# rclarey/torrent

Measured on AMD Instinct MI355X. Metric: verified GB/s (SHA-1 pieces, HBM-resident), higher is better.
Workload: dtype u32

## Files before the change

torrent_amd/csrc/tv_sha256.h:

```cpp
#pragma once
#include <stdint.h>

#if defined(__HIP_DEVICE_COMPILE__)
#define TV_SHA256_FN __device__ __forceinline__
#define TV_XOR3(a, b, c) __builtin_amdgcn_bitop3_b32((a), (b), (c), 0x96)
#define TV_CH(e, f, g) __builtin_amdgcn_bitop3_b32((e), (f), (g), 0xCA)
#define TV_MAJ(a, b, c) __builtin_amdgcn_bitop3_b32((a), (b), (c), 0xE8)
#define TV_ROR(x, n) __builtin_rotateright32((x), (n))
#else
#if defined(__HIPCC__)
#define TV_SHA256_FN __host__ __device__ inline
#else
#define TV_SHA256_FN inline
#endif
#define TV_XOR3(a, b, c) ((a) ^ (b) ^ (c))
#define TV_CH(e, f, g) (((e) & (f)) | (~(e) & (g)))
#define TV_MAJ(a, b, c) (((a) & (b)) | ((a) & (c)) | ((b) & (c)))
#define TV_ROR(x, n) (((x) >> (n)) | ((x) << (32 - (n))))
#endif

namespace tv256 {

constexpr uint32_t kK[64] = {
    0x428a2f98u, 0x71374491u, 0xb5c0fbcfu, 0xe9b5dba5u, 0x3956c25bu, 0x59f111f1u, 0x923f82a4u, 0xab1c5ed5u,
    0xd807aa98u, 0x12835b01u, 0x243185beu, 0x550c7dc3u, 0x72be5d74u, 0x80deb1feu, 0x9bdc06a7u, 0xc19bf174u,
    0xe49b69c1u, 0xefbe4786u, 0x0fc19dc6u, 0x240ca1ccu, 0x2de92c6fu, 0x4a7484aau, 0x5cb0a9dcu, 0x76f988dau,
    0x983e5152u, 0xa831c66du, 0xb00327c8u, 0xbf597fc7u, 0xc6e00bf3u, 0xd5a79147u, 0x06ca6351u, 0x14292967u,
    0x27b70a85u, 0x2e1b2138u, 0x4d2c6dfcu, 0x53380d13u, 0x650a7354u, 0x766a0abbu, 0x81c2c92eu, 0x92722c85u,
    0xa2bfe8a1u, 0xa81a664bu, 0xc24b8b70u, 0xc76c51a3u, 0xd192e819u, 0xd6990624u, 0xf40e3585u, 0x106aa070u,
    0x19a4c116u, 0x1e376c08u, 0x2748774cu, 0x34b0bcb5u, 0x391c0cb3u, 0x4ed8aa4au, 0x5b9cca4fu, 0x682e6ff3u,
    0x748f82eeu, 0x78a5636fu, 0x84c87814u, 0x8cc70208u, 0x90befffau, 0xa4506cebu, 0xbef9a3f7u, 0xc67178f2u};

TV_SHA256_FN void iv(uint32_t h[8]) {
    h[0] = 0x6a09e667u; h[1] = 0xbb67ae85u; h[2] = 0x3c6ef372u; h[3] = 0xa54ff53au;
    h[4] = 0x510e527fu; h[5] = 0x9b05688cu; h[6] = 0x1f83d9abu; h[7] = 0x5be0cd19u;
}

TV_SHA256_FN void compress(const uint32_t h[8], uint32_t w[16], uint32_t out[8]) {
    uint32_t a = h[0], b = h[1], c = h[2], d = h[3], e = h[4], f = h[5], g = h[6], hh = h[7];
#pragma unroll
    for (int t = 0; t < 64; t++) {
        if (t >= 16) {
            const uint32_t x = w[(t + 1) & 15], y = w[(t + 14) & 15];
            const uint32_t s0 = TV_XOR3(TV_ROR(x, 7), TV_ROR(x, 18), x >> 3);
            const uint32_t s1 = TV_XOR3(TV_ROR(y, 17), TV_ROR(y, 19), y >> 10);
            w[t & 15] = w[t & 15] + s0 + w[(t + 9) & 15] + s1;
        }
        const uint32_t S1 = TV_XOR3(TV_ROR(e, 6), TV_ROR(e, 11), TV_ROR(e, 25));
        const uint32_t S0 = TV_XOR3(TV_ROR(a, 2), TV_ROR(a, 13), TV_ROR(a, 22));
        const uint32_t t1 = hh + S1 + TV_CH(e, f, g) + kK[t] + w[t & 15];
        const uint32_t t2 = S0 + TV_MAJ(a, b, c);
        hh = g; g = f; f = e; e = d + t1; d = c; c = b; b = a; a = t1 + t2;
    }
    const uint32_t r[8] = {a, b, c, d, e, f, g, hh};
#pragma unroll
    for (int i = 0; i < 8; i++) out[i] = h[i] + r[i];
}

}
```

torrent_amd/csrc/tv_v2_kernels.hip:

```cpp
#include <hip/hip_runtime.h>
#include <stdint.h>

#include "tv_block.h"
#include "tv_internal.h"
#include "tv_sha256.h"

namespace {

constexpr uint32_t kLeaf = 16384;
constexpr int kDepth = 3;

__device__ __forceinline__ uint32_t wave_min(uint32_t v) {
#pragma unroll
    for (int m = 32; m >= 1; m >>= 1) {
        const uint32_t o = (uint32_t)__shfl_xor((int)v, m, 64);
        v = o < v ? o : v;
    }
    return (uint32_t)__builtin_amdgcn_readfirstlane((int)v);
}

__device__ __forceinline__ uint32_t wave_max(uint32_t v) {
#pragma unroll
    for (int m = 32; m >= 1; m >>= 1) {
        const uint32_t o = (uint32_t)__shfl_xor((int)v, m, 64);
        v = o > v ? o : v;
    }
    return (uint32_t)__builtin_amdgcn_readfirstlane((int)v);
}

__device__ __forceinline__ void bswap_block(const uint4 (&r)[4], uint32_t w[16]) {
#pragma unroll
    for (int i = 0; i < 4; i++) {
        w[4 * i + 0] = bswap32(r[i].x);
        w[4 * i + 1] = bswap32(r[i].y);
        w[4 * i + 2] = bswap32(r[i].z);
        w[4 * i + 3] = bswap32(r[i].w);
    }
}

__device__ __forceinline__ void hash_leaf(const uint8_t* leaf, uint32_t len, bool active, uint32_t h[8]) {
    const uint32_t nb = active ? (uint32_t)nblocks(len) : 0;
    const uint32_t fast_end = wave_min(active ? len >> 6 : 0xFFFFFFFFu);
    const uint32_t end = wave_max(nb);
    if (active) {
        uint32_t w[16];
        tv256::iv(h);
        uint32_t b = 0;
        if (b < fast_end) {
            const uint32_t last = fast_end - 1;
            uint4 R[kDepth][4];
#pragma unroll
            for (int d = 0; d < kDepth; d++) load_block(leaf, b + d < last ? b + d : last, R[d]);
            for (;;) {
#pragma unroll
                for (int d = 0; d < kDepth; d++) {
                    bswap_block(R[d], w);
                    load_block(leaf, b + kDepth < last ? b + kDepth : last, R[d]);
                    tv256::compress(h, w, h);
                    if (++b >= fast_end) goto raw_done;
                }
            }
        }
    raw_done:
        for (; b < end; b++) {
            build_tail_block(leaf, len, b, w);
            uint32_t r[8];
            tv256::compress(h, w, r);
            if (b < nb) {
#pragma unroll
                for (int i = 0; i < 8; i++) h[i] = r[i];
            }
        }
    }
}

__device__ __forceinline__ void hash_pair(uint32_t w[16], uint32_t h[8]) {
    tv256::iv(h);
    tv256::compress(h, w, h);
    uint32_t pad[16] = {0x80000000u, 0, 0, 0, 0, 0, 0, 0, 0, 0, 0, 0, 0, 0, 0, 512u};
    tv256::compress(h, pad, h);
}

}

template <int MAP>
__global__ __launch_bounds__(256) void tv_v2_leaf_kernel(TvV2 p) {
    uint64_t t0 = 0, r0 = 0;
    if (p.clock && blockIdx.x == 0) {
        t0 = __builtin_amdgcn_s_memtime();
        r0 = __builtin_amdgcn_s_memrealtime();
    }
    const uint32_t logW = p.logW, W = 1u << logW;
    const uint64_t t = (uint64_t)blockIdx.x * 256u + threadIdx.x;
    uint64_t j;
    uint32_t k;
    if (MAP == TV_V2_MAP_LEAF) {
        j = t >> logW;
        k = (uint32_t)t & (W - 1u);
    } else {
        const uint32_t r = (uint32_t)t & ((64u << logW) - 1u);
        j = (t >> (6u + logW)) * 64u + (r & 63u);
        k = r >> 6;
    }
    const bool valid = j < p.n;
    const uint64_t bytes = valid ? p.piece_bytes[j] : 0;
    const uint32_t wj = valid ? p.tree_leaves[j] : 0;
    const bool in_tree = k < wj;
    const uint64_t lo = (uint64_t)k * kLeaf;
    const bool active = in_tree && lo < bytes;
    const uint32_t len = active ? (uint32_t)(bytes - lo < kLeaf ? bytes - lo : kLeaf) : 0;
    const uint64_t np = (uint64_t)p.n << logW;
    const uint64_t slot = (j << logW) + k;
    if (in_tree && !active) {
#pragma unroll
        for (int q = 0; q < 8; q++) p.nodes_a[q * np + slot] = 0;
    }
    uint32_t h[8];
    hash_leaf(p.data + j * p.stride + lo, len, active, h);
    if (active) {
#pragma unroll
        for (int q = 0; q < 8; q++) p.nodes_a[q * np + slot] = h[q];
    }
    if (p.clock && blockIdx.x == 0 && threadIdx.x == 0) {
        const uint64_t t1 = __builtin_amdgcn_s_memtime(), r1 = __builtin_amdgcn_s_memrealtime();
        reinterpret_cast<ulonglong2*>(p.clock)[0] = make_ulonglong2(t0, r0);
        reinterpret_cast<ulonglong2*>(p.clock)[1] = make_ulonglong2(t1, r1);
    }
}

__global__ __launch_bounds__(256) void tv_v2_level_kernel(TvV2 p, uint32_t level, uint32_t log_half) {
    const uint64_t t = (uint64_t)blockIdx.x * 256u + threadIdx.x;
    const uint64_t j = t >> log_half;
    const uint32_t i = (uint32_t)t & ((1u << log_half) - 1u);
    if (j >= p.n) return;
    if (i >= (p.tree_leaves[j] >> (level + 1u))) return;
    const uint64_t W = 1ull << p.logW, WB = W > 1 ? W / 2 : 1;
    const bool from_a = (level & 1u) == 0;
    const uint32_t* in = from_a ? p.nodes_a : p.nodes_b;
    uint32_t* out = from_a ? p.nodes_b : p.nodes_a;
    const uint64_t in_row = from_a ? W : WB, out_row = from_a ? WB : W;
    const uint64_t in_np = p.n * in_row, out_np = p.n * out_row;
    const uint64_t src = j * in_row + 2ull * i, dst = j * out_row + i;
    uint32_t w[16], h[8];
#pragma unroll
    for (int q = 0; q < 8; q++) {
        const uint2 v = *reinterpret_cast<const uint2*>(in + q * in_np + src);
        w[q] = v.x;
        w[8 + q] = v.y;
    }
    tv256::iv(h);
    tv256::compress(h, w, h);
    uint32_t pad[16] = {0x80000000u, 0, 0, 0, 0, 0, 0, 0, 0, 0, 0, 0, 0, 0, 0, 512u};
    tv256::compress(h, pad, h);
#pragma unroll
    for (int q = 0; q < 8; q++) out[q * out_np + dst] = h[q];
}

template <bool HASH>
__global__ __launch_bounds__(256) void tv_v2_finish_kernel(TvV2 p) {
    const uint32_t j = blockIdx.x * 256u + threadIdx.x;
    bool ok = j < p.n;
    if (ok) {
        const uint64_t W = 1ull << p.logW, WB = W > 1 ? W / 2 : 1;
        const uint32_t lw = 31u - (uint32_t)__builtin_clz(p.tree_leaves[j]);
        const bool in_a = (lw & 1u) == 0;
        const uint32_t* src = in_a ? p.nodes_a : p.nodes_b;
        const uint64_t row = in_a ? W : WB, np = p.n * row;
#pragma unroll
        for (int q = 0; q < 8; q++) {
            const uint32_t v = src[q * np + j * row];
            if (HASH) p.roots[(uint64_t)q * p.n + j] = v;
            else ok &= v == p.expect[(uint64_t)q * p.n + j];
        }
    }
    if (HASH) return;
    const uint64_t mask = __ballot(ok);
    if ((threadIdx.x & 63u) == 0 && (p.out_words == 0 || (j >> 6) < p.out_words)) {
        uint64_t bits = __builtin_bswap64(__builtin_bitreverse64(mask));
        if (p.avail64) bits &= p.avail64[j >> 6];
        p.out64[j >> 6] = bits;
    }
}

namespace {

__device__ __forceinline__ void list_emit(const TvV2List& p, uint32_t e, const uint32_t h[8]) {
    bool ok = true;
#pragma unroll
    for (int q = 0; q < 8; q++) ok &= h[q] == p.expect[(uint64_t)q * p.m + e];
    p.out_bytes[e] = ok ? 1 : 0;
}

__device__ __forceinline__ bool list_level(uint32_t (&s)[8][256], uint32_t t, uint32_t parents, uint32_t h[8]) {
    const bool par = t < parents;
    uint32_t w[16];
    if (par) {
#pragma unroll
        for (int q = 0; q < 8; q++) {
            const uint2 v = *reinterpret_cast<const uint2*>(&s[q][2 * t]);
            w[q] = v.x;
            w[8 + q] = v.y;
        }
    }
    __syncthreads();
    if (par) {
        hash_pair(w, h);
#pragma unroll
        for (int q = 0; q < 8; q++) s[q][t] = h[q];
    }
    __syncthreads();
    return par;
}

}

template <bool TILED>
__global__ __launch_bounds__(256) void tv_v2_list_kernel(TvV2List p) {
    __shared__ __attribute__((aligned(16))) uint32_t s_node[8][256];
    __shared__ __attribute__((aligned(16))) uint32_t s_root[8][256];
    __shared__ uint32_t s_lw[256];
    const uint32_t t = threadIdx.x;
    const uint32_t logW = p.logW, logT = logW < 8u ? logW : 8u;
    const uint32_t tiles = 1u << (logW - logT);
    const uint32_t e0 = blockIdx.x << (8u - logT);
    const uint32_t e = e0 + (t >> logT), kt = t & ((1u << logT) - 1u);
    const bool valid = e < p.m;
    const uint32_t bytes = valid ? p.bytes[e] : 0;
    const uint32_t we = valid ? p.widths[e] : 0;
    const uint8_t* row = p.data + (valid ? (uint64_t)p.rows[e] * p.stride : 0);
    if (kt == 0) s_lw[t >> logT] = valid ? 31u - (uint32_t)__builtin_clz(we) : 0xFFu;
    uint32_t h[8];
    for (uint32_t T = 0; T < (TILED ? tiles : 1u); T++) {
        const uint32_t k = (T << logT) + kt;
        const uint32_t lo = k * kLeaf;
        const bool active = k < we && lo < bytes;
        const uint32_t len = active ? (bytes - lo < kLeaf ? bytes - lo : kLeaf) : 0;
        hash_leaf(row + lo, len, active, h);
        if (!active) {
#pragma unroll
            for (int q = 0; q < 8; q++) h[q] = 0;
        }
        if (T == 0 && kt == 0 && we == 1) list_emit(p, e, h);
#pragma unroll
        for (int q = 0; q < 8; q++) s_node[q][t] = h[q];
        __syncthreads();
        for (uint32_t l = 0; l < logT; l++) {
            if (!list_level(s_node, t, 256u >> (l + 1u), h)) continue;
            const uint32_t sh = logT - l - 1u, g = t >> sh;
            if ((t & ((1u << sh) - 1u)) != 0) continue;
            if (T == 0 && s_lw[g] == l + 1u) list_emit(p, e0 + g, h);
            if (tiles > 1 && sh == 0) {
#pragma unroll
                for (int q = 0; q < 8; q++) s_root[q][T] = h[q];
            }
        }
    }
    if (TILED) __syncthreads();
    for (uint32_t l = 8; l < logW; l++)
        if (list_level(s_root, t, tiles >> (l - 7u), h) && t == 0 && s_lw[0] == l + 1u) list_emit(p, e0, h);
}

namespace {

__device__ __forceinline__ void column_store(const TvV2Col& p, uint32_t j, const uint32_t h[8]) {
    const uint64_t np = (uint64_t)p.n << p.logn, slot = ((uint64_t)j << p.logn) + p.col;
#pragma unroll
    for (int q = 0; q < 8; q++) p.nodes[q * np + slot] = h[q];
}

}

template <bool TILED>
__global__ __launch_bounds__(256) void tv_v2_column_kernel(TvV2Col p) {
    __shared__ __attribute__((aligned(16))) uint32_t s_node[8][256];
    __shared__ __attribute__((aligned(16))) uint32_t s_root[8][256];
    __shared__ uint32_t s_tg[256];
    uint64_t t0 = 0, r0 = 0;
    if (p.clock && blockIdx.x == 0) {
        t0 = __builtin_amdgcn_s_memtime();
        r0 = __builtin_amdgcn_s_memrealtime();
    }
    const uint32_t t = threadIdx.x;
    const uint32_t logc = p.logc, logT = logc < 8u ? logc : 8u;
    const uint32_t tiles = 1u << (logc - logT);
    const uint32_t j0 = blockIdx.x << (8u - logT);
    const uint32_t j = j0 + (t >> logT), kt = t & ((1u << logT) - 1u);
    const bool valid = j < p.n;
    const uint32_t bytes = valid ? p.piece_bytes[j] : 0;
    const uint32_t wj = valid ? p.tree_leaves[j] : 0;
    const uint64_t k0 = (uint64_t)p.col << logc;
    const bool reach = k0 < wj;
    const uint32_t lw = wj ? 31u - (uint32_t)__builtin_clz(wj) : 0u;
    const uint32_t target = lw < logc ? lw : logc;
    const uint8_t* row = p.data + (valid ? (uint64_t)j * p.stride : 0);
    if (kt == 0) s_tg[t >> logT] = reach ? target : 0xFFu;
    uint32_t h[8];
    for (uint32_t T = 0; T < (TILED ? tiles : 1u); T++) {
        const uint32_t kr = (T << logT) + kt;
        const uint64_t lo = (k0 + kr) * kLeaf;
        const bool active = k0 + kr < wj && lo < bytes;
        const uint32_t len = active ? (uint32_t)(bytes - lo < kLeaf ? bytes - lo : kLeaf) : 0;
        hash_leaf(row + (uint64_t)kr * kLeaf, len, active, h);
        if (!active) {
#pragma unroll
            for (int q = 0; q < 8; q++) h[q] = 0;
        }
        if (T == 0 && kt == 0 && reach && target == 0) column_store(p, j, h);
#pragma unroll
        for (int q = 0; q < 8; q++) s_node[q][t] = h[q];
        __syncthreads();
        for (uint32_t l = 0; l < logT; l++) {
            if (!list_level(s_node, t, 256u >> (l + 1u), h)) continue;
            const uint32_t sh = logT - l - 1u, g = t >> sh;
            if ((t & ((1u << sh) - 1u)) != 0) continue;
            if (T == 0 && s_tg[g] == l + 1u) column_store(p, j0 + g, h);
            if (tiles > 1 && sh == 0) {
#pragma unroll
                for (int q = 0; q < 8; q++) s_root[q][T] = h[q];
            }
        }
    }
    if (TILED) __syncthreads();
    for (uint32_t l = 8; l < logc; l++)
        if (list_level(s_root, t, tiles >> (l - 7u), h) && t == 0 && s_tg[0] == l + 1u) column_store(p, j0, h);
    if (p.clock && blockIdx.x == 0 && threadIdx.x == 0) {
        const uint64_t t1 = __builtin_amdgcn_s_memtime(), r1 = __builtin_amdgcn_s_memrealtime();
        reinterpret_cast<ulonglong2*>(p.clock)[0] = make_ulonglong2(t0, r0);
        reinterpret_cast<ulonglong2*>(p.clock)[1] = make_ulonglong2(t1, r1);
    }
}

template <bool CHECK>
__global__ __launch_bounds__(256) void tv_v2_block_kernel(TvV2Blocks p) {
    const uint32_t t = blockIdx.x * 256u + threadIdx.x;
    const bool active = t < p.m;
    const uint32_t row = active ? p.rows[t] : 0;
    const uint32_t leaf = active ? p.leaves[t] : 0;
    const uint32_t len = active ? p.lens[t] : 0;
    uint32_t h[8];
    hash_leaf(p.data + (uint64_t)row * p.stride + (uint64_t)leaf * kLeaf, len, active, h);
    if (CHECK) {
        bool ok = active;
        if (active) {
#pragma unroll
            for (int q = 0; q < 8; q++) ok &= h[q] == p.expect[(uint64_t)q * p.m + t];
        }
        const uint64_t mask = __ballot(ok);
        if ((threadIdx.x & 63u) == 0 && active) p.out64[t >> 6] = mask;
    } else if (active) {
#pragma unroll
        for (int q = 0; q < 8; q++) p.hashes[(uint64_t)q * p.m + t] = h[q];
    }
}

hipError_t tv_v2_launch_blocks(const TvV2Blocks& p, bool check, hipStream_t s, uint32_t* workgroups) {
    if (workgroups) *workgroups = 0;
    if (p.m == 0) return hipSuccess;
    if (p.m > TV_V2_BLOCKS_MAX_ITEMS) return hipErrorInvalidValue;
    const uint32_t grid = (p.m + 255u) / 256u;
    if (workgroups) *workgroups = grid;
    if (check) hipLaunchKernelGGL(tv_v2_block_kernel<true>, dim3(grid), dim3(256), 0, s, p);
    else hipLaunchKernelGGL(tv_v2_block_kernel<false>, dim3(grid), dim3(256), 0, s, p);
    return hipGetLastError();
}

hipError_t tv_v2_launch_column(const TvV2Col& p, hipStream_t s, uint32_t* workgroups) {
    if (workgroups) *workgroups = 0;
    if (p.n == 0) return hipSuccess;
    if (p.logc > TV_V2_COL_MAX_LOGC || (p.col >> p.logn) != 0) return hipErrorInvalidValue;
    const uint32_t logG = p.logc < 8u ? 8u - p.logc : 0u;
    const uint64_t grid = (((uint64_t)p.n - 1) >> logG) + 1;
    if (grid > 0x7FFFFFFFull) return hipErrorInvalidConfiguration;
    if (workgroups) *workgroups = (uint32_t)grid;
    if (p.logc > 8u) hipLaunchKernelGGL(tv_v2_column_kernel<true>, dim3((unsigned)grid), dim3(256), 0, s, p);
    else hipLaunchKernelGGL(tv_v2_column_kernel<false>, dim3((unsigned)grid), dim3(256), 0, s, p);
    return hipGetLastError();
}

hipError_t tv_v2_launch_leaves(const TvV2& p, hipStream_t s, uint32_t* workgroups) {
    if (workgroups) *workgroups = 0;
    if (p.n == 0) return hipSuccess;
    const uint64_t pieces = p.map == TV_V2_MAP_PIECE ? ((uint64_t)p.n + 63) / 64 * 64 : p.n;
    const uint64_t grid = ((pieces << p.logW) + 255) / 256;
    if (grid > 0x7FFFFFFFull) return hipErrorInvalidConfiguration;
    if (workgroups) *workgroups = (uint32_t)grid;
    if (p.map == TV_V2_MAP_PIECE)
        hipLaunchKernelGGL((tv_v2_leaf_kernel<TV_V2_MAP_PIECE>), dim3((unsigned)grid), dim3(256), 0, s, p);
    else
        hipLaunchKernelGGL((tv_v2_leaf_kernel<TV_V2_MAP_LEAF>), dim3((unsigned)grid), dim3(256), 0, s, p);
    return hipGetLastError();
}

hipError_t tv_v2_launch_level(const TvV2& p, uint32_t level, uint32_t maxlog, hipStream_t s) {
    if (p.n == 0 || level >= maxlog) return hipSuccess;
    const uint32_t log_half = maxlog - level - 1;
    const uint64_t grid = (((uint64_t)p.n << log_half) + 255) / 256;
    if (grid > 0x7FFFFFFFull) return hipErrorInvalidConfiguration;
    hipLaunchKernelGGL(tv_v2_level_kernel, dim3((unsigned)grid), dim3(256), 0, s, p, level, log_half);
    return hipGetLastError();
}

hipError_t tv_v2_launch_list(const TvV2List& p, hipStream_t s, uint32_t* workgroups) {
    if (workgroups) *workgroups = 0;
    if (p.m == 0) return hipSuccess;
    if (p.logW > TV_V2_LIST_MAX_LOGW) return hipErrorInvalidValue;
    const uint32_t logG = p.logW < 8u ? 8u - p.logW : 0u;
    const uint64_t grid = (((uint64_t)p.m - 1) >> logG) + 1;
    if (grid > 0x7FFFFFFFull) return hipErrorInvalidConfiguration;
    if (workgroups) *workgroups = (uint32_t)grid;
    if (p.logW > 8u) hipLaunchKernelGGL(tv_v2_list_kernel<true>, dim3((unsigned)grid), dim3(256), 0, s, p);
    else hipLaunchKernelGGL(tv_v2_list_kernel<false>, dim3((unsigned)grid), dim3(256), 0, s, p);
    return hipGetLastError();
}

hipError_t tv_v2_launch_finish(const TvV2& p, bool hash, hipStream_t s) {
    if (p.n == 0) return hipSuccess;
    const dim3 grid((p.n + 255) / 256);
    if (hash) hipLaunchKernelGGL((tv_v2_finish_kernel<true>), grid, dim3(256), 0, s, p);
    else hipLaunchKernelGGL((tv_v2_finish_kernel<false>), grid, dim3(256), 0, s, p);
    return hipGetLastError();
}
```

Before: 1442.

## Add lean single-buffer SHA-256 leaf path with in-round prefetch and occupancy hint

Adds a compress_lean variant that byte-swaps message words inside the first 16 rounds and issues the next block's load after round 15, once the raw registers are free. This lets the leaf kernel hold one block of prefetch instead of three. The leaf kernel defaults to depth 1 with a waves-per-EU attribute of 7, trading prefetch depth for more resident waves to hide HBM latency. Per-round asm fences and sched_barriers pin the instruction schedule, which may stop the compiler from interleaving work across rounds. The leaf-map slot index is also simplified to the thread id.

```diff
diff --git a/torrent_amd/csrc/tv_sha256.h b/torrent_amd/csrc/tv_sha256.h
--- a/torrent_amd/csrc/tv_sha256.h
+++ b/torrent_amd/csrc/tv_sha256.h
@@ -7,6 +7,11 @@
 #define TV_CH(e, f, g) __builtin_amdgcn_bitop3_b32((e), (f), (g), 0xCA)
 #define TV_MAJ(a, b, c) __builtin_amdgcn_bitop3_b32((a), (b), (c), 0xE8)
 #define TV_ROR(x, n) __builtin_rotateright32((x), (n))
+#define TV_ROUND_FENCE(a, e, w)                        \
+    do {                                               \
+        asm volatile("" : "+v"(a), "+v"(e), "+v"(w));  \
+        __builtin_amdgcn_sched_barrier(0);             \
+    } while (0)
 #else
 #if defined(__HIPCC__)
 #define TV_SHA256_FN __host__ __device__ inline
@@ -17,7 +22,9 @@
 #define TV_CH(e, f, g) (((e) & (f)) | (~(e) & (g)))
 #define TV_MAJ(a, b, c) (((a) & (b)) | ((a) & (c)) | ((b) & (c)))
 #define TV_ROR(x, n) (((x) >> (n)) | ((x) << (32 - (n))))
+#define TV_ROUND_FENCE(a, e, w) ((void)0)
 #endif
+#define TV_BSWAP(x) __builtin_bswap32(x)
 
 namespace tv256 {
 
@@ -57,4 +64,28 @@
     for (int i = 0; i < 8; i++) out[i] = h[i] + r[i];
 }
 
+template <bool SWAP, class After16>
+TV_SHA256_FN void compress_lean(uint32_t h[8], const uint32_t raw[16], uint32_t w[16], After16 after16) {
+    uint32_t a = h[0], b = h[1], c = h[2], d = h[3], e = h[4], f = h[5], g = h[6], hh = h[7];
+#pragma unroll
+    for (int t = 0; t < 64; t++) {
+        if (t < 16) {
+            w[t] = SWAP ? TV_BSWAP(raw[t]) : raw[t];
+        } else {
+            const uint32_t x = w[(t + 1) & 15], y = w[(t + 14) & 15];
+            const uint32_t s0 = TV_XOR3(TV_ROR(x, 7), TV_ROR(x, 18), x >> 3);
+            const uint32_t s1 = TV_XOR3(TV_ROR(y, 17), TV_ROR(y, 19), y >> 10);
+            w[t & 15] = w[t & 15] + s0 + w[(t + 9) & 15] + s1;
+        }
+        const uint32_t S1 = TV_XOR3(TV_ROR(e, 6), TV_ROR(e, 11), TV_ROR(e, 25));
+        const uint32_t S0 = TV_XOR3(TV_ROR(a, 2), TV_ROR(a, 13), TV_ROR(a, 22));
+        const uint32_t t1 = hh + S1 + TV_CH(e, f, g) + kK[t] + w[t & 15];
+        const uint32_t t2 = S0 + TV_MAJ(a, b, c);
+        hh = g; g = f; f = e; e = d + t1; d = c; c = b; b = a; a = t1 + t2;
+        if (t == 15) after16();
+        TV_ROUND_FENCE(a, e, w[t < 15 ? t : (t + 1) & 15]);
+    }
+    h[0] += a; h[1] += b; h[2] += c; h[3] += d; h[4] += e; h[5] += f; h[6] += g; h[7] += hh;
 }
+
+}
diff --git a/torrent_amd/csrc/tv_v2_kernels.hip b/torrent_amd/csrc/tv_v2_kernels.hip
--- a/torrent_amd/csrc/tv_v2_kernels.hip
+++ b/torrent_amd/csrc/tv_v2_kernels.hip
@@ -8,7 +8,17 @@
 namespace {
 
 constexpr uint32_t kLeaf = 16384;
-constexpr int kDepth = 3;
+#ifndef TV_V2_LEAF_DEPTH
+#define TV_V2_LEAF_DEPTH 1
+#endif
+#ifndef TV_V2_LEAF_WAVES
+#define TV_V2_LEAF_WAVES 7
+#endif
+#define TV_V2_WAVES __attribute__((amdgpu_waves_per_eu(TV_V2_LEAF_WAVES, TV_V2_LEAF_WAVES)))
+constexpr int kDepth = TV_V2_LEAF_DEPTH;
+constexpr int kWaves = TV_V2_LEAF_WAVES;
+constexpr int kListDepth = 3;
+static_assert(kDepth >= 1 && kDepth <= 3 && kWaves >= 1 && kWaves <= 8, "TV_V2_LEAF_DEPTH 1..3, TV_V2_LEAF_WAVES 1..8");
 
 __device__ __forceinline__ uint32_t wave_min(uint32_t v) {
 #pragma unroll
@@ -38,6 +48,7 @@
     }
 }
 
+template <int DEPTH>
 __device__ __forceinline__ void hash_leaf(const uint8_t* leaf, uint32_t len, bool active, uint32_t h[8]) {
     const uint32_t nb = active ? (uint32_t)nblocks(len) : 0;
     const uint32_t fast_end = wave_min(active ? len >> 6 : 0xFFFFFFFFu);
@@ -48,24 +59,43 @@
         uint32_t b = 0;
         if (b < fast_end) {
             const uint32_t last = fast_end - 1;
-            uint4 R[kDepth][4];
-#pragma unroll
-            for (int d = 0; d < kDepth; d++) load_block(leaf, b + d < last ? b + d : last, R[d]);
-            for (;;) {
-#pragma unroll
-                for (int d = 0; d < kDepth; d++) {
-                    bswap_block(R[d], w);
-                    load_block(leaf, b + kDepth < last ? b + kDepth : last, R[d]);
-                    tv256::compress(h, w, h);
-                    if (++b >= fast_end) goto raw_done;
+            if constexpr (DEPTH == 1) {
+                uint4 R[4];
+                load_block(leaf, 0, R);
+                const uint8_t* next = leaf;
+                do {
+                    next += b < last ? 64 : 0;
+                    tv256::compress_lean<true>(h, reinterpret_cast<const uint32_t*>(R), w,
+                                               [&] { load_block(next, 0, R); });
+                } while (++b < fast_end);
+            } else {
+                uint4 R[DEPTH][4];
+#pragma unroll
+                for (int d = 0; d < DEPTH; d++) load_block(leaf, b + d < last ? b + d : last, R[d]);
+                for (;;) {
+#pragma unroll
+                    for (int d = 0; d < DEPTH; d++) {
+                        bswap_block(R[d], w);
+                        load_block(leaf, b + DEPTH < last ? b + DEPTH : last, R[d]);
+                        tv256::compress(h, w, h);
+                        if (++b >= fast_end) goto raw_done;
+                    }
                 }
             }
         }
     raw_done:
         for (; b < end; b++) {
-            build_tail_block(leaf, len, b, w);
             uint32_t r[8];
-            tv256::compress(h, w, r);
+            if constexpr (DEPTH == 1) {
+                uint32_t tw[16];
+                build_tail_block(leaf, len, b, tw);
+#pragma unroll
+                for (int i = 0; i < 8; i++) r[i] = h[i];
+                tv256::compress_lean<false>(r, tw, w, [] {});
+            } else {
+                build_tail_block(leaf, len, b, w);
+                tv256::compress(h, w, r);
+            }
             if (b < nb) {
 #pragma unroll
                 for (int i = 0; i < 8; i++) h[i] = r[i];
@@ -84,7 +114,7 @@
 }
 
 template <int MAP>
-__global__ __launch_bounds__(256) void tv_v2_leaf_kernel(TvV2 p) {
+__global__ __launch_bounds__(256) TV_V2_WAVES void tv_v2_leaf_kernel(TvV2 p) {
     uint64_t t0 = 0, r0 = 0;
     if (p.clock && blockIdx.x == 0) {
         t0 = __builtin_amdgcn_s_memtime();
@@ -110,13 +140,13 @@
     const bool active = in_tree && lo < bytes;
     const uint32_t len = active ? (uint32_t)(bytes - lo < kLeaf ? bytes - lo : kLeaf) : 0;
     const uint64_t np = (uint64_t)p.n << logW;
-    const uint64_t slot = (j << logW) + k;
+    const uint64_t slot = MAP == TV_V2_MAP_LEAF ? t : (j << logW) + k;
     if (in_tree && !active) {
 #pragma unroll
         for (int q = 0; q < 8; q++) p.nodes_a[q * np + slot] = 0;
     }
     uint32_t h[8];
-    hash_leaf(p.data + j * p.stride + lo, len, active, h);
+    hash_leaf<kDepth>(p.data + j * p.stride + lo, len, active, h);
     if (active) {
 #pragma unroll
         for (int q = 0; q < 8; q++) p.nodes_a[q * np + slot] = h[q];
@@ -235,7 +265,7 @@
         const uint32_t lo = k * kLeaf;
         const bool active = k < we && lo < bytes;
         const uint32_t len = active ? (bytes - lo < kLeaf ? bytes - lo : kLeaf) : 0;
-        hash_leaf(row + lo, len, active, h);
+        hash_leaf<kListDepth>(row + lo, len, active, h);
         if (!active) {
 #pragma unroll
             for (int q = 0; q < 8; q++) h[q] = 0;
@@ -300,7 +330,7 @@
         const uint64_t lo = (k0 + kr) * kLeaf;
         const bool active = k0 + kr < wj && lo < bytes;
         const uint32_t len = active ? (uint32_t)(bytes - lo < kLeaf ? bytes - lo : kLeaf) : 0;
-        hash_leaf(row + (uint64_t)kr * kLeaf, len, active, h);
+        hash_leaf<kListDepth>(row + (uint64_t)kr * kLeaf, len, active, h);
         if (!active) {
 #pragma unroll
             for (int q = 0; q < 8; q++) h[q] = 0;
@@ -338,7 +368,7 @@
     const uint32_t leaf = active ? p.leaves[t] : 0;
     const uint32_t len = active ? p.lens[t] : 0;
     uint32_t h[8];
-    hash_leaf(p.data + (uint64_t)row * p.stride + (uint64_t)leaf * kLeaf, len, active, h);
+    hash_leaf<kListDepth>(p.data + (uint64_t)row * p.stride + (uint64_t)leaf * kLeaf, len, active, h);
     if (CHECK) {
         bool ok = active;
         if (active) {
```

Result: no change. 1443 (median of 2 runs) (+0.1%).
